# zju3dv/OnePose_Plus_Plus

Measured on AMD Instinct MI355X. Metric: query images/sec (2D-3D match fwd) at 512x512 img x 5k pts, higher is better.
Workload: dtype f32 (operands as exact bf16 triples, f32 accumulate)

## Files before the change

### onepose_plus_plus_amd/csrc/enc_layer64.hip

```cpp
#include <stdlib.h>

#include <type_traits>

#include "enc_frag.h"

namespace {

constexpr int R64 = 64, C = 256, NW = 8, NT = 512, D = 32;
constexpr int SA = a_stride_bytes(C);
constexpr int SS = C + 4;
constexpr int OFF_S = R64 * SA, OFF_Z = OFF_S + 32 * SS * 4;
constexpr size_t kLds64 = OFF_Z + 1024;

__global__ __launch_bounds__(NT) void enc_layer64_kernel(const OppEncChain a) {
  extern __shared__ __attribute__((aligned(16))) char smem[];
  char* A = smem;
  float* S = reinterpret_cast<float*>(smem + OFF_S);
  float* z_sh = reinterpret_cast<float*>(smem + OFF_Z);

  const int tid = threadIdx.x, lane = tid & 63;
  const int wave = __builtin_amdgcn_readfirstlane(tid >> 6);
  const int half = lane >> 5, l31 = lane & 31;

  const int chunks0 = (a.len0 + R64 - 1) / R64;
  const int stream = (int)blockIdx.x >= chunks0 ? 1 : 0;
  const int cidx = stream ? blockIdx.x - chunks0 : blockIdx.x;
  const int seg_len = stream ? a.len1 : a.len0;
  const int row0 = (stream ? a.len0 : 0) + cidx * R64;
  const int nrows = min(R64, seg_len - cidx * R64);
  const float* qrows = (stream && a.q1 != nullptr) ? a.q1 + (size_t)(cidx * R64) * a.ldq : a.q + (size_t)row0 * a.ldq;

  const char* a_lane = A + l31 * SA + half * 48;
  auto gemm = [&](auto ntile_c, auto depth_c, auto s0_c, auto s1_c, auto ks_c, const void* wf, int t0, f32x16 (&acc)[2][decltype(ntile_c)::value], int tstep = 1) {
    constexpr int NTILE = decltype(ntile_c)::value, DEPTH = decltype(depth_c)::value;
    constexpr int S0 = decltype(s0_c)::value, S1 = decltype(s1_c)::value, KS = decltype(ks_c)::value;
    constexpr int NSTEP = S1 - S0;
    const __amdgpu_buffer_rsrc_t rsrc = __builtin_amdgcn_make_buffer_rsrc(const_cast<void*>(wf), 0, 0x7fffffff, 0x00020000);
    const int voff = lane * 16;
    u32x4 bq[DEPTH][NTILE][3];
    u32x4 af[2][2][3];
    auto load_b = [&](int s, int slot) {
#pragma unroll
      for (int j = 0; j < NTILE; ++j)
#pragma unroll
        for (int p = 0; p < 3; ++p)
          bq[slot][j][p] = __builtin_amdgcn_raw_buffer_load_b128(rsrc, voff, (((t0 + j * tstep) * KS + S0 + s) * 3 + p) * 1024, 0);
    };
    auto load_a = [&](int s, int slot) {
#pragma unroll
      for (int i = 0; i < 2; ++i)
#pragma unroll
        for (int q = 0; q < 3; ++q) af[slot][i][q] = *reinterpret_cast<const u32x4*>(a_lane + i * 32 * SA + s * 96 + q * 16);
    };
#pragma unroll
    for (int s = 0; s < DEPTH && s < NSTEP; ++s) load_b(s, s);
    load_a(0, 0);
    __builtin_amdgcn_sched_barrier(0);
    constexpr int PA[6] = {2, 0, 1, 1, 0, 0};
    constexpr int PB[6] = {0, 2, 1, 0, 1, 0};
#pragma unroll
    for (int s = 0; s < NSTEP; ++s) {
      if (s + 1 < NSTEP) load_a(s + 1, (s + 1) & 1);
#pragma unroll
      for (int pr = 0; pr < 6; ++pr)
#pragma unroll
        for (int i = 0; i < 2; ++i)
#pragma unroll
          for (int j = 0; j < NTILE; ++j)
            acc[i][j] = __builtin_amdgcn_mfma_f32_32x32x16_bf16(__builtin_bit_cast(bf16x8, af[s & 1][i][PA[pr]]),
                                                                 __builtin_bit_cast(bf16x8, bq[s % DEPTH][j][PB[pr]]), acc[i][j], 0, 0, 0);
      if (s + DEPTH < NSTEP) load_b(s + DEPTH, s % DEPTH);
      __builtin_amdgcn_sched_barrier(0);
    }
  };
  auto ic = [](auto v) { return v; };
  (void)ic;
  auto stage = [&](const f32x16& t, int col0, bool relu) {
#pragma unroll
    for (int r = 0; r < 16; ++r) {
      const int row = (r & 3) + 8 * (r >> 2) + 4 * half;
      float v = t[r];
      if (relu) v = v < 0.f ? 0.f : v;
      S[row * SS + col0 + l31] = v;
    }
  };
  auto split_staged = [&](int rb, int g0) {
#pragma unroll
    for (int i = 0; i < 32 * (C / 8) / NT; ++i) {
      const int p = tid + i * NT;
      const int r = p / (C / 8), g = p - r * (C / 8);
      const float4* s4 = reinterpret_cast<const float4*>(S + r * SS + g * 8);
      split8_store(s4[0], s4[1], A + (rb + r) * SA + (g0 + g) * 48);
    }
  };
  typedef float vec_t __attribute__((ext_vector_type(4)));
  auto layernorm_rows = [&](const float* gamma, const float* beta, float eps, auto mode_c, int rb) {
    constexpr int MODE = decltype(mode_c)::value;
    const vec_t gmv = *reinterpret_cast<const vec_t*>(gamma + lane * 4);
    const vec_t btv = *reinterpret_cast<const vec_t*>(beta + lane * 4);
    constexpr int RPW = 32 / NW;
    float v[RPW][4], sm[RPW], mean[RPW], rstd[RPW];
#pragma unroll
    for (int r = 0; r < RPW; ++r) {
      const vec_t t = *reinterpret_cast<const vec_t*>(S + (wave * RPW + r) * SS + lane * 4);
      sm[r] = 0.f;
#pragma unroll
      for (int i = 0; i < 4; ++i) {
        v[r][i] = t[i];
        sm[r] += t[i];
      }
    }
#pragma unroll
    for (int r = 0; r < RPW; ++r) sm[r] = opp_wave_sum_dpp(sm[r]);
#pragma unroll
    for (int r = 0; r < RPW; ++r) {
      mean[r] = sm[r] / (float)C;
      sm[r] = 0.f;
#pragma unroll
      for (int i = 0; i < 4; ++i) {
        const float d = v[r][i] - mean[r];
        sm[r] = opp_ln_sq_acc(d, sm[r]);
      }
    }
#pragma unroll
    for (int r = 0; r < RPW; ++r) sm[r] = opp_wave_sum_dpp(sm[r]);
#pragma unroll
    for (int r = 0; r < RPW; ++r) rstd[r] = 1.0f / sqrtf(sm[r] / (float)C + eps);
#pragma unroll
    for (int r = 0; r < RPW; ++r) {
      const int lr = rb + wave * RPW + r;
      float y[4];
#pragma unroll
      for (int i = 0; i < 4; ++i) y[i] = opp_ln_affine(v[r][i], mean[r], rstd[r], gmv[i], btv[i]);
      if constexpr (MODE != 0) {
        if (lr < nrows) {
          const vec_t xr = *reinterpret_cast<const vec_t*>(a.X + (size_t)(row0 + lr) * a.ldx + lane * 4);
          vec_t o;
#pragma unroll
          for (int i = 0; i < 4; ++i) o[i] = xr[i] + y[i];
          *reinterpret_cast<vec_t*>(a.out + (size_t)(row0 + lr) * a.ldo + lane * 4) = o;
#pragma unroll
          for (int i = 0; i < 4; ++i) y[i] = o[i];
        } else {
#pragma unroll
          for (int i = 0; i < 4; ++i) y[i] = 0.f;
        }
      }
      if constexpr (MODE != 1) {
        char* g = A + lr * SA + ((lane * 4) >> 3) * 48 + ((lane * 4) & 7) * 2;
#pragma unroll
        for (int i = 0; i < 4; i += 2) {
          unsigned hi, mid, lo;
          split2(y[i], y[i + 1], hi, mid, lo);
          *reinterpret_cast<unsigned*>(g + i * 2) = hi;
          *reinterpret_cast<unsigned*>(g + 16 + i * 2) = mid;
          *reinterpret_cast<unsigned*>(g + 32 + i * 2) = lo;
        }
      }
    }
  };
  auto zero2 = [](auto& acc) {
#pragma unroll
    for (auto& row : acc)
#pragma unroll
      for (auto& t : row)
#pragma unroll
        for (int r = 0; r < 16; ++r) t[r] = 0.f;
  };
  using I0 = std::integral_constant<int, 0>;
  using I1 = std::integral_constant<int, 1>;
  using I2 = std::integral_constant<int, 2>;
  using I3 = std::integral_constant<int, 3>;
  using I4 = std::integral_constant<int, 4>;
  using I16 = std::integral_constant<int, 16>;
  using I32 = std::integral_constant<int, 32>;

#pragma unroll
  for (int i = 0; i < R64 * (C / 8) / NT; ++i) {
    const int p = tid + i * NT;
    const int r = p / (C / 8), g = p - r * (C / 8);
    float4 v0 = make_float4(0.f, 0.f, 0.f, 0.f), v1 = v0;
    if (r < nrows) {
      const float4* s4 = reinterpret_cast<const float4*>(a.X + (size_t)(row0 + r) * a.ldx + g * 8);
      v0 = s4[0];
      v1 = s4[1];
    }
    split8_store(v0, v1, A + r * SA + g * 48);
  }
  const int src = a.cross ? 1 - stream : stream;
  const float src_len = (float)(src ? a.len1 : a.len0);
  const float* kvp = (src && a.kv1 != nullptr) ? a.kv1 : a.kv + (size_t)src * (C * D);
  const float* ksp = (src && a.ks1 != nullptr) ? a.ks1 : a.ks + (size_t)src * C;
  const int h = wave;
  float bk[16];
#pragma unroll
  for (int i = 0; i < 16; ++i) bk[i] = kvp[(h * D + 2 * i + half) * D + l31];
  __syncthreads();
  f32x16 hid[2][2];
  zero2(hid);
  gemm(I2{}, I3{}, I0{}, I16{}, I32{}, a.w1, wave * 2, hid);
  __syncthreads();

  constexpr int QS = 258;
  float* qsh = S;
#pragma unroll
  for (int rh = 0; rh < 2; ++rh) {
#pragma unroll
    for (int i = 0; i < 32 * (C / 4) / NT; ++i) {
      const int e = tid + i * NT;
      const int r = e / (C / 4), c4 = e - r * (C / 4);
      float4 q = make_float4(0.f, 0.f, 0.f, 0.f);
      if (rh * 32 + r < nrows) q = *reinterpret_cast<const float4*>(qrows + (size_t)(rh * 32 + r) * a.ldq + c4 * 4);
      float2* dst = reinterpret_cast<float2*>(qsh + r * QS + c4 * 4);
      dst[0] = make_float2(q.x, q.y);
      dst[1] = make_float2(q.z, q.w);
    }
    __syncthreads();
    if (tid < 8 * 32) {
      const int tok = tid & 31, hh = tid >> 5;
      const float* q = qsh + tok * QS + hh * D;
      const float* k = ksp + hh * D;
      float den = 0.f;
#pragma unroll
      for (int d = 0; d < D; ++d) den = fmaf(q[d], k[d], den);
      z_sh[hh * 32 + tok] = 1.0f / (den + a.eps_attn);
    }
    f32x16 num;
#pragma unroll
    for (int r = 0; r < 16; ++r) num[r] = 0.f;
#pragma unroll
    for (int i = 0; i < 16; ++i) num = __builtin_amdgcn_mfma_f32_32x32x2f32(qsh[l31 * QS + h * D + 2 * i + half], bk[i], num, 0, 0, 0);
    __syncthreads();
    {
      char* col = A + (h * 4 + (l31 >> 3)) * 48 + (l31 & 7) * 2;
#pragma unroll
      for (int r = 0; r < 16; ++r) {
        const int row = (r & 3) + 8 * (r >> 2) + 4 * half;
        const float v = (num[r] * z_sh[h * 32 + row]) * src_len;
        unsigned hi, mid, lo;
        split2(v, 0.f, hi, mid, lo);
        char* d = col + (rh * 32 + row) * SA;
        *reinterpret_cast<unsigned short*>(d) = (unsigned short)hi;
        *reinterpret_cast<unsigned short*>(d + 16) = (unsigned short)mid;
        *reinterpret_cast<unsigned short*>(d + 32) = (unsigned short)lo;
      }
    }
    __syncthreads();
  }

  {
    f32x16 acc[2][1];
    zero2(acc);
    gemm(I1{}, I4{}, I0{}, I16{}, I16{}, a.wm, wave, acc);
    __syncthreads();
#pragma unroll
    for (int rh = 0; rh < 2; ++rh) {
      stage(acc[rh][0], wave * 32, false);
      __syncthreads();
      layernorm_rows(a.g1, a.b1, a.eps_ln, I0{}, rh * 32);
      __syncthreads();
    }
  }

  gemm(I2{}, I3{}, I16{}, I32{}, I32{}, a.w1, wave * 2, hid);
  __syncthreads();

  f32x16 out[2][1];
  zero2(out);
#pragma unroll
  for (int kh = 0; kh < 2; ++kh) {
#pragma unroll
    for (int rh = 0; rh < 2; ++rh) {
      if (wave / (NW / 2) == kh) {
        const int c0 = (wave - kh * (NW / 2)) * 64;
        stage(hid[rh][0], c0, true);
        stage(hid[rh][1], c0 + 32, true);
      }
      __syncthreads();
      split_staged(rh * 32, 0);
      __syncthreads();
    }
    if (kh == 0) gemm(I1{}, I4{}, I0{}, I16{}, I32{}, a.w2, wave, out);
    else gemm(I1{}, I4{}, I16{}, I32{}, I32{}, a.w2, wave, out);
    __syncthreads();
  }

  const bool fold = a.wq_next != nullptr;
#pragma unroll
  for (int rh = 0; rh < 2; ++rh) {
    stage(out[rh][0], wave * 32, false);
    __syncthreads();
    if (fold) layernorm_rows(a.g2, a.b2, a.eps_ln, I2{}, rh * 32);
    else layernorm_rows(a.g2, a.b2, a.eps_ln, I1{}, rh * 32);
    __syncthreads();
  }
  if (!fold) return;

  float* qdst = (stream && a.qkv_out1 != nullptr) ? a.qkv_out1 + (size_t)(cidx * R64) * (3 * C) : a.qkv_out + (size_t)row0 * (3 * C);
  const float vdiv = (float)seg_len;
  auto finish_qkv = [&](f32x16& t, int rb, bool qk) {
#pragma unroll
    for (int r = 0; r < 16; ++r) {
      const int row = rb + (r & 3) + 8 * (r >> 2) + 4 * half;
      float v = 0.f;
      if (row < nrows) {
        v = t[r];
        if (qk) v = v > 0.f ? v + 1.f : __expf(v);
        else v = v / vdiv;
        if (stream == 0 && a.qmask != nullptr) v *= a.qmask[row0 + row];
      }
      t[r] = v;
    }
  };
  auto store_qkv = [&](const f32x16& t, int rb, int tile) {
    const int col = tile * 32 + l31;
#pragma unroll
    for (int r = 0; r < 16; ++r) {
      const int row = rb + (r & 3) + 8 * (r >> 2) + 4 * half;
      if (row < nrows) qdst[(size_t)row * (3 * C) + col] = t[r];
    }
  };
  const bool kv_fold = a.kv_part != nullptr;
  {
    f32x16 acc[2][1];
    zero2(acc);
    gemm(I1{}, I4{}, I0{}, I16{}, I16{}, a.wq_next, h, acc);
#pragma unroll
    for (int i = 0; i < 2; ++i) {
      finish_qkv(acc[i][0], i * 32, true);
      store_qkv(acc[i][0], i * 32, h);
    }
  }
  f32x16 acc[2][2];
  zero2(acc);
  gemm(I2{}, I3{}, I0{}, I16{}, I16{}, a.wq_next, NW + h, acc, NW);
#pragma unroll
  for (int i = 0; i < 2; ++i) {
    finish_qkv(acc[i][0], i * 32, true);
    finish_qkv(acc[i][1], i * 32, false);
  }
  if (!kv_fold) {
#pragma unroll
    for (int i = 0; i < 2; ++i) {
      store_qkv(acc[i][0], i * 32, NW + h);
      store_qkv(acc[i][1], i * 32, 2 * NW + h);
    }
    return;
  }
  {
    f32x16 kvacc;
#pragma unroll
    for (int r = 0; r < 16; ++r) kvacc[r] = 0.f;
    float ksum = 0.f;
    auto swap = [](float x, float y, float& lo, float& hi) {
      const auto r = __builtin_amdgcn_permlane32_swap(__builtin_bit_cast(unsigned, x), __builtin_bit_cast(unsigned, y), false, false);
      lo = __builtin_bit_cast(float, (unsigned)r[0]);
      hi = __builtin_bit_cast(float, (unsigned)r[1]);
    };
#pragma unroll
    for (int i = 0; i < 2; ++i)
#pragma unroll
      for (int q = 0; q < 4; ++q) {
        float kk[2][2], vv[2][2];
#pragma unroll
        for (int e = 0; e < 2; ++e) {
          swap(acc[i][0][4 * q + 2 * e], acc[i][0][4 * q + 2 * e + 1], kk[0][e], kk[1][e]);
          swap(acc[i][1][4 * q + 2 * e], acc[i][1][4 * q + 2 * e + 1], vv[0][e], vv[1][e]);
        }
#pragma unroll
        for (int g = 0; g < 2; ++g)
#pragma unroll
          for (int e = 0; e < 2; ++e) {
            kvacc = __builtin_amdgcn_mfma_f32_32x32x2f32(kk[g][e], vv[g][e], kvacc, 0, 0, 0);
            ksum += kk[g][e];
          }
      }
    float* kvp = a.kv_part + (size_t)blockIdx.x * (C * D) + h * (D * D);
#pragma unroll
    for (int r = 0; r < 16; ++r) {
      const int d = (r & 3) + 8 * (r >> 2) + 4 * half;
      kvp[d * D + l31] = kvacc[r];
    }
    const float tot = ksum + __shfl_xor(ksum, 32, 64);
    if (half == 0) a.ks_part[(size_t)blockIdx.x * C + h * D + l31] = tot;
  }
}

}

int opp_enc_layer64(const OppEncChain& a, hipStream_t stream) {
  OPP_CHECK_ARG(a.C == 256 && a.apply && a.X && a.out && a.q && a.kv && a.ks && a.wm && a.w1 && a.w2 && a.g1 && a.b1 && a.g2 && a.b2,
                "enc_layer64: coarse level (C = 256) with the fused attention apply only");
  OPP_CHECK_ARG(a.len0 >= 0 && a.len1 >= 0 && a.len0 + a.len1 > 0, "enc_layer64: empty token set");
  auto al16 = [](const void* p) { return (reinterpret_cast<uintptr_t>(p) & 15) == 0; };
  OPP_CHECK_ARG(al16(a.X) && al16(a.out) && al16(a.q) && a.ldx % 4 == 0 && a.ldo % 4 == 0 && a.ldq % 4 == 0 && al16(a.g1) && al16(a.b1) &&
                    al16(a.g2) && al16(a.b2) && al16(a.wm) && al16(a.w1) && al16(a.w2) && al16(a.q1), "enc_layer64: operands must be 16-byte aligned");
  OPP_CHECK_ARG(a.wq_next == nullptr || (a.qkv_out != nullptr && al16(a.wq_next)), "enc_layer64: folded projection needs its output buffer");
  OPP_CHECK_ARG((a.kv_part == nullptr) == (a.ks_part == nullptr) && (a.kv_part == nullptr || (a.wq_next != nullptr && a.qkv_out1 == nullptr)),
                "enc_layer64: the KV partials need the folded projection and both of their buffers");
  static OppLdsOnce lds_once;
  opp_lds_opt_in(reinterpret_cast<const void*>(enc_layer64_kernel), kLds64, lds_once);
  const int tiles = opp_cdiv(a.len0, R64) + opp_cdiv(a.len1, R64);
  OppProfScope prof(OPP_PROF_ENC_CHAIN, stream, 2.0 * (double)(a.len0 + a.len1) * ((a.wq_next ? 10.0 : 7.0) * C * C + 32.0 * C));
  hipLaunchKernelGGL(enc_layer64_kernel, dim3(tiles), dim3(NT), kLds64, stream, a);
  OPP_CHECK_LAUNCH("enc_layer64_kernel");
  return OPP_OK;
}
```

Measured before the change: 599.4.

## Prefetch weight rings across phases and stage LN params, ks, mask in LDS

Weight tiles for each GEMM are now preloaded into a register ring during the preceding phase (barriers, layernorm, epilogue) instead of at GEMM start, hiding global-load latency behind other work. X and Q rows and the residual X are loaded into registers early, and LN gamma/beta, the ks vector and the query mask are staged once into shared memory so later phases read from LDS. Boundary-row predicates are simplified with clamped indices and fast paths for full tiles. This raises register and LDS pressure, which may lower occupancy, and adds an optional cycle-stamp instrumentation path behind a tuning macro.

After: 599.9 (median of 6 runs). About the same (+0.1%).

```diff
diff --git a/onepose_plus_plus_amd/csrc/enc_layer64.hip b/onepose_plus_plus_amd/csrc/enc_layer64.hip
--- a/onepose_plus_plus_amd/csrc/enc_layer64.hip
+++ b/onepose_plus_plus_amd/csrc/enc_layer64.hip
@@ -10,14 +10,39 @@
 constexpr int SA = a_stride_bytes(C);
 constexpr int SS = C + 4;
 constexpr int OFF_S = R64 * SA, OFF_Z = OFF_S + 32 * SS * 4;
-constexpr size_t kLds64 = OFF_Z + 1024;
+constexpr int OFF_LN = OFF_Z + 1024;
+constexpr int OFF_M = OFF_LN + 5 * C * 4;
+constexpr size_t kLds64 = OFF_M + R64 * 4;
+constexpr int kWaitVm0 = 0x0F70;
+
+template <int DEPTH_, int NTILE_>
+struct WRing {
+  static constexpr int DEPTH = DEPTH_, NTILE = NTILE_;
+  u32x4 q[DEPTH_][NTILE_][3];
+};
+
+#ifdef OPP_TUNING
+constexpr int kStamps = 16, kStampBlocks = 512;
+__device__ unsigned long long enc64_stamps[kStampBlocks * NW * kStamps];
+#define OPP_ENC64_STAMP(i) ts[i] = __builtin_readcyclecounter()
+#else
+#define OPP_ENC64_STAMP(i)
+#endif
 
 __global__ __launch_bounds__(NT) void enc_layer64_kernel(const OppEncChain a) {
+#ifdef OPP_TUNING
+  unsigned long long ts[kStamps] = {};
+#endif
+  OPP_ENC64_STAMP(0);
   extern __shared__ __attribute__((aligned(16))) char smem[];
   char* A = smem;
   float* S = reinterpret_cast<float*>(smem + OFF_S);
   float* z_sh = reinterpret_cast<float*>(smem + OFF_Z);
-
+  float* ln_sh = reinterpret_cast<float*>(smem + OFF_LN);
+  const float* ks_sh = ln_sh + 4 * C;
+  float* mask_sh = reinterpret_cast<float*>(smem + OFF_M);
+
+  typedef float vec_t __attribute__((ext_vector_type(4)));
   const int tid = threadIdx.x, lane = tid & 63;
   const int wave = __builtin_amdgcn_readfirstlane(tid >> 6);
   const int half = lane >> 5, l31 = lane & 31;
@@ -31,13 +56,27 @@
   const float* qrows = (stream && a.q1 != nullptr) ? a.q1 + (size_t)(cidx * R64) * a.ldq : a.q + (size_t)row0 * a.ldq;
 
   const char* a_lane = A + l31 * SA + half * 48;
-  auto gemm = [&](auto ntile_c, auto depth_c, auto s0_c, auto s1_c, auto ks_c, const void* wf, int t0, f32x16 (&acc)[2][decltype(ntile_c)::value], int tstep = 1) {
-    constexpr int NTILE = decltype(ntile_c)::value, DEPTH = decltype(depth_c)::value;
+  auto ring_load = [&](auto& ring, auto s0_c, auto ks_c, const void* wf, int t0, int tstep = 1) {
+    using R = std::remove_reference_t<decltype(ring)>;
+    constexpr int S0 = decltype(s0_c)::value, KS = decltype(ks_c)::value;
+    const __amdgpu_buffer_rsrc_t rsrc = __builtin_amdgcn_make_buffer_rsrc(const_cast<void*>(wf), 0, 0x7fffffff, 0x00020000);
+#pragma unroll
+    for (int s = 0; s < R::DEPTH; ++s)
+#pragma unroll
+      for (int j = 0; j < R::NTILE; ++j)
+#pragma unroll
+        for (int p = 0; p < 3; ++p)
+          ring.q[s][j][p] = __builtin_amdgcn_raw_buffer_load_b128(rsrc, lane * 16, (((t0 + j * tstep) * KS + S0 + s) * 3 + p) * 1024, 0);
+    __builtin_amdgcn_sched_barrier(0);
+  };
+  auto gemm = [&](auto& ring, auto s0_c, auto s1_c, auto ks_c, const void* wf, int t0, f32x16 (&acc)[2][std::remove_reference_t<decltype(ring)>::NTILE], int tstep = 1) {
+    constexpr int NTILE = std::remove_reference_t<decltype(ring)>::NTILE, DEPTH = std::remove_reference_t<decltype(ring)>::DEPTH;
     constexpr int S0 = decltype(s0_c)::value, S1 = decltype(s1_c)::value, KS = decltype(ks_c)::value;
     constexpr int NSTEP = S1 - S0;
+    static_assert(NSTEP >= DEPTH, "the preloaded ring holds DEPTH steps");
     const __amdgpu_buffer_rsrc_t rsrc = __builtin_amdgcn_make_buffer_rsrc(const_cast<void*>(wf), 0, 0x7fffffff, 0x00020000);
     const int voff = lane * 16;
-    u32x4 bq[DEPTH][NTILE][3];
+    auto& bq = ring.q;
     u32x4 af[2][2][3];
     auto load_b = [&](int s, int slot) {
 #pragma unroll
@@ -52,8 +91,6 @@
 #pragma unroll
         for (int q = 0; q < 3; ++q) af[slot][i][q] = *reinterpret_cast<const u32x4*>(a_lane + i * 32 * SA + s * 96 + q * 16);
     };
-#pragma unroll
-    for (int s = 0; s < DEPTH && s < NSTEP; ++s) load_b(s, s);
     load_a(0, 0);
     __builtin_amdgcn_sched_barrier(0);
     constexpr int PA[6] = {2, 0, 1, 1, 0, 0};
@@ -93,12 +130,22 @@
       split8_store(s4[0], s4[1], A + (rb + r) * SA + (g0 + g) * 48);
     }
   };
-  typedef float vec_t __attribute__((ext_vector_type(4)));
+  constexpr int RPW = 32 / NW;
+  vec_t xres[2][RPW];
+  auto load_xres = [&]() {
+#pragma unroll
+    for (int rh = 0; rh < 2; ++rh)
+#pragma unroll
+      for (int r = 0; r < RPW; ++r) {
+        const int lr = min(rh * 32 + wave * RPW + r, nrows - 1);
+        xres[rh][r] = *reinterpret_cast<const vec_t*>(a.X + (size_t)(row0 + lr) * a.ldx + lane * 4);
+      }
+    __builtin_amdgcn_sched_barrier(0);
+  };
   auto layernorm_rows = [&](const float* gamma, const float* beta, float eps, auto mode_c, int rb) {
     constexpr int MODE = decltype(mode_c)::value;
     const vec_t gmv = *reinterpret_cast<const vec_t*>(gamma + lane * 4);
     const vec_t btv = *reinterpret_cast<const vec_t*>(beta + lane * 4);
-    constexpr int RPW = 32 / NW;
     float v[RPW][4], sm[RPW], mean[RPW], rstd[RPW];
 #pragma unroll
     for (int r = 0; r < RPW; ++r) {
@@ -133,8 +180,8 @@
 #pragma unroll
       for (int i = 0; i < 4; ++i) y[i] = opp_ln_affine(v[r][i], mean[r], rstd[r], gmv[i], btv[i]);
       if constexpr (MODE != 0) {
-        if (lr < nrows) {
-          const vec_t xr = *reinterpret_cast<const vec_t*>(a.X + (size_t)(row0 + lr) * a.ldx + lane * 4);
+        if (__builtin_amdgcn_readfirstlane(lr) < nrows) {
+          const vec_t xr = xres[rb >> 5][r];
           vec_t o;
 #pragma unroll
           for (int i = 0; i < 4; ++i) o[i] = xr[i] + y[i];
@@ -170,56 +217,84 @@
   using I0 = std::integral_constant<int, 0>;
   using I1 = std::integral_constant<int, 1>;
   using I2 = std::integral_constant<int, 2>;
-  using I3 = std::integral_constant<int, 3>;
-  using I4 = std::integral_constant<int, 4>;
   using I16 = std::integral_constant<int, 16>;
   using I32 = std::integral_constant<int, 32>;
 
-#pragma unroll
-  for (int i = 0; i < R64 * (C / 8) / NT; ++i) {
+  const int h = wave;
+  WRing<3, 2> ring_w1;
+  ring_load(ring_w1, I0{}, I32{}, a.w1, wave * 2);
+  constexpr int XI = R64 * (C / 8) / NT;
+  float4 xv[XI][2];
+#pragma unroll
+  for (int i = 0; i < XI; ++i) {
     const int p = tid + i * NT;
     const int r = p / (C / 8), g = p - r * (C / 8);
-    float4 v0 = make_float4(0.f, 0.f, 0.f, 0.f), v1 = v0;
-    if (r < nrows) {
-      const float4* s4 = reinterpret_cast<const float4*>(a.X + (size_t)(row0 + r) * a.ldx + g * 8);
-      v0 = s4[0];
-      v1 = s4[1];
-    }
-    split8_store(v0, v1, A + r * SA + g * 48);
-  }
+    const float4* s4 = reinterpret_cast<const float4*>(a.X + (size_t)(row0 + min(r, nrows - 1)) * a.ldx + g * 8);
+    xv[i][0] = s4[0];
+    xv[i][1] = s4[1];
+  }
+  constexpr int QI = 32 * (C / 4) / NT;
+  constexpr int QS = 258;
+  float* qsh = S;
+  float4 qv[QI];
+  auto load_q = [&](int rh) {
+#pragma unroll
+    for (int i = 0; i < QI; ++i)
+      qv[i] = *reinterpret_cast<const float4*>(qrows + (size_t)min(rh * 32 + wave + 8 * i, nrows - 1) * a.ldq + lane * 4);
+  };
+  auto put_q = [&](int rh) {
+#pragma unroll
+    for (int i = 0; i < QI; ++i) {
+      const int r = wave + 8 * i;
+      const bool in = rh * 32 + r < nrows;
+      float2* dst = reinterpret_cast<float2*>(qsh + r * QS + lane * 4);
+      dst[0] = make_float2(in ? qv[i].x : 0.f, in ? qv[i].y : 0.f);
+      dst[1] = make_float2(in ? qv[i].z : 0.f, in ? qv[i].w : 0.f);
+    }
+  };
+  load_q(0);
   const int src = a.cross ? 1 - stream : stream;
   const float src_len = (float)(src ? a.len1 : a.len0);
   const float* kvp = (src && a.kv1 != nullptr) ? a.kv1 : a.kv + (size_t)src * (C * D);
   const float* ksp = (src && a.ks1 != nullptr) ? a.ks1 : a.ks + (size_t)src * C;
-  const int h = wave;
   float bk[16];
 #pragma unroll
   for (int i = 0; i < 16; ++i) bk[i] = kvp[(h * D + 2 * i + half) * D + l31];
+  const int lnw = wave < 5 ? wave : wave & 3;
+  const float* lnp = lnw == 4 ? ksp : (lnw & 2) ? ((lnw & 1) ? a.b2 : a.g2) : ((lnw & 1) ? a.b1 : a.g1);
+  const vec_t lnv = *reinterpret_cast<const vec_t*>(lnp + lane * 4);
+  const bool masked = stream == 0 && a.qmask != nullptr;
+  float mv = 1.f;
+  if (masked) mv = a.qmask[row0 + min(lane, nrows - 1)];
+  __builtin_amdgcn_sched_barrier(0);
+#pragma unroll
+  for (int i = 0; i < XI; ++i) {
+    const int p = tid + i * NT;
+    const int r = p / (C / 8), g = p - r * (C / 8);
+    const float4 z4 = make_float4(0.f, 0.f, 0.f, 0.f);
+    split8_store(r < nrows ? xv[i][0] : z4, r < nrows ? xv[i][1] : z4, A + r * SA + g * 48);
+  }
+  put_q(0);
+  *reinterpret_cast<vec_t*>(ln_sh + lnw * C + lane * 4) = lnv;
+  mask_sh[lane] = mv;
+  OPP_ENC64_STAMP(1);
   __syncthreads();
   f32x16 hid[2][2];
   zero2(hid);
-  gemm(I2{}, I3{}, I0{}, I16{}, I32{}, a.w1, wave * 2, hid);
+  gemm(ring_w1, I0{}, I16{}, I32{}, a.w1, wave * 2, hid);
+  OPP_ENC64_STAMP(2);
   __syncthreads();
 
-  constexpr int QS = 258;
-  float* qsh = S;
+  WRing<4, 1> ring_m;
+  ring_load(ring_m, I0{}, I16{}, a.wm, wave);
+  load_q(1);
+  __builtin_amdgcn_sched_barrier(0);
 #pragma unroll
   for (int rh = 0; rh < 2; ++rh) {
-#pragma unroll
-    for (int i = 0; i < 32 * (C / 4) / NT; ++i) {
-      const int e = tid + i * NT;
-      const int r = e / (C / 4), c4 = e - r * (C / 4);
-      float4 q = make_float4(0.f, 0.f, 0.f, 0.f);
-      if (rh * 32 + r < nrows) q = *reinterpret_cast<const float4*>(qrows + (size_t)(rh * 32 + r) * a.ldq + c4 * 4);
-      float2* dst = reinterpret_cast<float2*>(qsh + r * QS + c4 * 4);
-      dst[0] = make_float2(q.x, q.y);
-      dst[1] = make_float2(q.z, q.w);
-    }
-    __syncthreads();
     if (tid < 8 * 32) {
       const int tok = tid & 31, hh = tid >> 5;
       const float* q = qsh + tok * QS + hh * D;
-      const float* k = ksp + hh * D;
+      const float* k = ks_sh + hh * D;
       float den = 0.f;
 #pragma unroll
       for (int d = 0; d < D; ++d) den = fmaf(q[d], k[d], den);
@@ -245,30 +320,39 @@
         *reinterpret_cast<unsigned short*>(d + 32) = (unsigned short)lo;
       }
     }
+    if (rh == 0) put_q(1);
     __syncthreads();
   }
 
+  OPP_ENC64_STAMP(3);
   {
     f32x16 acc[2][1];
     zero2(acc);
-    gemm(I1{}, I4{}, I0{}, I16{}, I16{}, a.wm, wave, acc);
+    gemm(ring_m, I0{}, I16{}, I16{}, a.wm, wave, acc);
+    OPP_ENC64_STAMP(4);
+    ring_load(ring_w1, I16{}, I32{}, a.w1, wave * 2);
     __syncthreads();
 #pragma unroll
     for (int rh = 0; rh < 2; ++rh) {
       stage(acc[rh][0], wave * 32, false);
       __syncthreads();
-      layernorm_rows(a.g1, a.b1, a.eps_ln, I0{}, rh * 32);
+      layernorm_rows(ln_sh, ln_sh + C, a.eps_ln, I0{}, rh * 32);
       __syncthreads();
     }
   }
 
-  gemm(I2{}, I3{}, I16{}, I32{}, I32{}, a.w1, wave * 2, hid);
+  OPP_ENC64_STAMP(5);
+  gemm(ring_w1, I16{}, I32{}, I32{}, a.w1, wave * 2, hid);
+  OPP_ENC64_STAMP(6);
   __syncthreads();
 
   f32x16 out[2][1];
   zero2(out);
 #pragma unroll
   for (int kh = 0; kh < 2; ++kh) {
+    if (kh == 0) ring_load(ring_m, I0{}, I32{}, a.w2, wave);
+    else ring_load(ring_m, I16{}, I32{}, a.w2, wave);
+    if (kh == 1) load_xres();
 #pragma unroll
     for (int rh = 0; rh < 2; ++rh) {
       if (wave / (NW / 2) == kh) {
@@ -280,40 +364,48 @@
       split_staged(rh * 32, 0);
       __syncthreads();
     }
-    if (kh == 0) gemm(I1{}, I4{}, I0{}, I16{}, I32{}, a.w2, wave, out);
-    else gemm(I1{}, I4{}, I16{}, I32{}, I32{}, a.w2, wave, out);
+    OPP_ENC64_STAMP(7 + 2 * kh);
+    if (kh == 0) gemm(ring_m, I0{}, I16{}, I32{}, a.w2, wave, out);
+    else gemm(ring_m, I16{}, I32{}, I32{}, a.w2, wave, out);
+    OPP_ENC64_STAMP(8 + 2 * kh);
     __syncthreads();
   }
 
   const bool fold = a.wq_next != nullptr;
+  __builtin_amdgcn_s_waitcnt(kWaitVm0);
+  if (fold) ring_load(ring_m, I0{}, I16{}, a.wq_next, h);
 #pragma unroll
   for (int rh = 0; rh < 2; ++rh) {
     stage(out[rh][0], wave * 32, false);
     __syncthreads();
-    if (fold) layernorm_rows(a.g2, a.b2, a.eps_ln, I2{}, rh * 32);
-    else layernorm_rows(a.g2, a.b2, a.eps_ln, I1{}, rh * 32);
+    if (fold) layernorm_rows(ln_sh + 2 * C, ln_sh + 3 * C, a.eps_ln, I2{}, rh * 32);
+    else layernorm_rows(ln_sh + 2 * C, ln_sh + 3 * C, a.eps_ln, I1{}, rh * 32);
     __syncthreads();
   }
+  OPP_ENC64_STAMP(11);
   if (!fold) return;
 
   float* qdst = (stream && a.qkv_out1 != nullptr) ? a.qkv_out1 + (size_t)(cidx * R64) * (3 * C) : a.qkv_out + (size_t)row0 * (3 * C);
   const float vdiv = (float)seg_len;
   auto finish_qkv = [&](f32x16& t, int rb, bool qk) {
+    const bool whole = nrows - rb >= 32;
 #pragma unroll
     for (int r = 0; r < 16; ++r) {
       const int row = rb + (r & 3) + 8 * (r >> 2) + 4 * half;
-      float v = 0.f;
-      if (row < nrows) {
-        v = t[r];
-        if (qk) v = v > 0.f ? v + 1.f : __expf(v);
-        else v = v / vdiv;
-        if (stream == 0 && a.qmask != nullptr) v *= a.qmask[row0 + row];
-      }
-      t[r] = v;
+      float v = t[r];
+      if (qk) v = v > 0.f ? v + 1.f : __expf(v);
+      else v = v / vdiv;
+      if (masked) v *= mask_sh[row];
+      t[r] = (whole || row < nrows) ? v : 0.f;
     }
   };
   auto store_qkv = [&](const f32x16& t, int rb, int tile) {
     const int col = tile * 32 + l31;
+    if (nrows - rb >= 32) {
+#pragma unroll
+      for (int r = 0; r < 16; ++r) qdst[(size_t)(rb + (r & 3) + 8 * (r >> 2) + 4 * half) * (3 * C) + col] = t[r];
+      return;
+    }
 #pragma unroll
     for (int r = 0; r < 16; ++r) {
       const int row = rb + (r & 3) + 8 * (r >> 2) + 4 * half;
@@ -324,7 +416,9 @@
   {
     f32x16 acc[2][1];
     zero2(acc);
-    gemm(I1{}, I4{}, I0{}, I16{}, I16{}, a.wq_next, h, acc);
+    gemm(ring_m, I0{}, I16{}, I16{}, a.wq_next, h, acc);
+    OPP_ENC64_STAMP(12);
+    ring_load(ring_w1, I0{}, I16{}, a.wq_next, NW + h, NW);
 #pragma unroll
     for (int i = 0; i < 2; ++i) {
       finish_qkv(acc[i][0], i * 32, true);
@@ -333,7 +427,9 @@
   }
   f32x16 acc[2][2];
   zero2(acc);
-  gemm(I2{}, I3{}, I0{}, I16{}, I16{}, a.wq_next, NW + h, acc, NW);
+  OPP_ENC64_STAMP(13);
+  gemm(ring_w1, I0{}, I16{}, I16{}, a.wq_next, NW + h, acc, NW);
+  OPP_ENC64_STAMP(14);
 #pragma unroll
   for (int i = 0; i < 2; ++i) {
     finish_qkv(acc[i][0], i * 32, true);
@@ -384,6 +480,11 @@
     const float tot = ksum + __shfl_xor(ksum, 32, 64);
     if (half == 0) a.ks_part[(size_t)blockIdx.x * C + h * D + l31] = tot;
   }
+#ifdef OPP_TUNING
+  OPP_ENC64_STAMP(15);
+  if (lane == 0 && blockIdx.x < kStampBlocks)
+    for (int i = 0; i < kStamps; ++i) enc64_stamps[((size_t)blockIdx.x * NW + wave) * kStamps + i] = ts[i];
+#endif
 }
 
 }
@@ -394,15 +495,43 @@
   OPP_CHECK_ARG(a.len0 >= 0 && a.len1 >= 0 && a.len0 + a.len1 > 0, "enc_layer64: empty token set");
   auto al16 = [](const void* p) { return (reinterpret_cast<uintptr_t>(p) & 15) == 0; };
   OPP_CHECK_ARG(al16(a.X) && al16(a.out) && al16(a.q) && a.ldx % 4 == 0 && a.ldo % 4 == 0 && a.ldq % 4 == 0 && al16(a.g1) && al16(a.b1) &&
-                    al16(a.g2) && al16(a.b2) && al16(a.wm) && al16(a.w1) && al16(a.w2) && al16(a.q1), "enc_layer64: operands must be 16-byte aligned");
+                    al16(a.g2) && al16(a.b2) && al16(a.ks) && al16(a.ks1) && al16(a.wm) && al16(a.w1) && al16(a.w2) && al16(a.q1), "enc_layer64: operands must be 16-byte aligned");
   OPP_CHECK_ARG(a.wq_next == nullptr || (a.qkv_out != nullptr && al16(a.wq_next)), "enc_layer64: folded projection needs its output buffer");
   OPP_CHECK_ARG((a.kv_part == nullptr) == (a.ks_part == nullptr) && (a.kv_part == nullptr || (a.wq_next != nullptr && a.qkv_out1 == nullptr)),
                 "enc_layer64: the KV partials need the folded projection and both of their buffers");
+  {
+    const size_t T = (size_t)a.len0 + (size_t)a.len1;
+    const float* xe = a.X + (T - 1) * (size_t)a.ldx + C;
+    const float* oe = a.out + (T - 1) * (size_t)a.ldo + C;
+    const bool in_place = a.out == a.X && a.ldo == a.ldx;
+    const bool apart = reinterpret_cast<uintptr_t>(oe) <= reinterpret_cast<uintptr_t>(a.X) || reinterpret_cast<uintptr_t>(xe) <= reinterpret_cast<uintptr_t>(a.out);
+    OPP_CHECK_ARG(a.ldx >= C && a.ldo >= C && (in_place || apart), "enc_layer64: out and X may only overlap as out == X with ldo == ldx");
+  }
   static OppLdsOnce lds_once;
   opp_lds_opt_in(reinterpret_cast<const void*>(enc_layer64_kernel), kLds64, lds_once);
   const int tiles = opp_cdiv(a.len0, R64) + opp_cdiv(a.len1, R64);
   OppProfScope prof(OPP_PROF_ENC_CHAIN, stream, 2.0 * (double)(a.len0 + a.len1) * ((a.wq_next ? 10.0 : 7.0) * C * C + 32.0 * C));
   hipLaunchKernelGGL(enc_layer64_kernel, dim3(tiles), dim3(NT), kLds64, stream, a);
   OPP_CHECK_LAUNCH("enc_layer64_kernel");
+#ifdef OPP_TUNING
+  static const bool stamps = getenv("OPP_ENC64_STAMPS") != nullptr;
+  static int printed = 0;
+  if (stamps && a.kv_part != nullptr && printed < 4 && hipStreamSynchronize(stream) == hipSuccess) {
+    static unsigned long long host[kStampBlocks * NW * kStamps];
+    const int nb = tiles < kStampBlocks ? tiles : kStampBlocks;
+    if (hipMemcpyFromSymbol(host, HIP_SYMBOL(enc64_stamps), sizeof(host)) == hipSuccess) {
+      ++printed;
+      fprintf(stderr, "enc_layer64 stamps, %d tiles, mean shader-clock cycles per phase over tiles and waves:", nb);
+      double total = 0.0;
+      for (int i = 1; i < kStamps; ++i) {
+        double sum = 0.0;
+        for (int t = 0; t < nb * NW; ++t) sum += (double)(host[t * kStamps + i] - host[t * kStamps + i - 1]);
+        fprintf(stderr, " %d:%.0f", i, sum / (nb * NW));
+        total += sum / (nb * NW);
+      }
+      fprintf(stderr, " total:%.0f\n", total);
+    }
+  }
+#endif
   return OPP_OK;
 }
```
